# lzhangbj/deep_video_interpolation_extrapolation

Measured on AMD Instinct MI355X. Metric: train frames/s (256x512 len-3 clips), higher is better.
Workload: dtype bf16; 1 GPU; InterNet int_5_len_3 train step 256x512 bf16; per_gpu_batch=8, global_batch=8, parallelism=dp1, step=eager, executor side-stream lanes

## Files before the change

deep_video_interpolation_extrapolation_amd/csrc/conv.hip:

```cpp
#include <cxxabi.h>
#include <dlfcn.h>
#include <stdarg.h>
#include <stdio.h>
#include <stdlib.h>
#include <string.h>

#include <string>
#include <vector>

#include "common.h"

namespace dvie {

static thread_local char g_err[512];
void set_error(const char* fmt, ...) {
  va_list ap;
  va_start(ap, fmt);
  vsnprintf(g_err, sizeof(g_err), fmt, ap);
  va_end(ap);
}
const char* last_error() { return g_err; }

thread_local bool g_trace_on = false;
static thread_local std::vector<const void*> g_trace;
// ... 330 lines not shown
    for (int e = 0; e < 4; ++e) red[tid * 4 + e] = s[e];
    __syncthreads();
    if (tid < 256 / nrl && qb + tid < cq) {
      f32x4 t = f32x4{0.f, 0.f, 0.f, 0.f};
      for (int k = 0; k < nrl; ++k)
        for (int e = 0; e < 4; ++e) t[e] += red[(k * (256 / nrl) + tid) * 4 + e];
      for (int e = 0; e < 4; ++e) p.ws[(long long)blockIdx.x * p.c + 4 * (qb + tid) + e] = t[e];
    }
    __syncthreads();
  }
}

enum { PACK_ELEM = 0, PACK_ROW = 1, PACK_TILE = 2 };
constexpr int PACK_LDS = 8192;
constexpr int PACK_TR = 8, PACK_TC = 64;

__host__ __device__ inline int pack_kind(const dvie_pack_desc& d) {
  if (d.kpad < 64 || d.kpad % 4 != 0) return PACK_ELEM;
  if (d.mode == 0 && d.cin_s * d.kh_s * d.kw_s <= PACK_LDS) return PACK_ROW;
  if (d.mode == 1 && d.kh_s * d.kw_s <= 16 && d.c % 4 == 0) return PACK_TILE;
  return PACK_ELEM;
}

__device__ __forceinline__ void pack_store4(const dvie_pack_desc& p, long long e, const float* v) {
  if (p.dtype == DVIE_BF16) {
    uint2 u;
    u.x = (uint32_t)f2bf(v[0]) | ((uint32_t)f2bf(v[1]) << 16);
    u.y = (uint32_t)f2bf(v[2]) | ((uint32_t)f2bf(v[3]) << 16);
    *(uint2*)((bf16_t*)p.dst + e) = u;
  } else {
    *(f32x4*)((float*)p.dst + e) = f32x4{v[0], v[1], v[2], v[3]};
  }
}

__global__ __launch_bounds__(256) void pack_kernel(const dvie_pack_desc* __restrict__ descs, int n) {
  __shared__ float lds[PACK_LDS];
  int lo = 0, hi = n - 1;
  const int b = blockIdx.x;
  while (lo < hi) {
    const int mid = (lo + hi + 1) >> 1;
    if (descs[mid].blk0 <= b)
      lo = mid;
    else
      hi = mid - 1;
  }
  const dvie_pack_desc p = descs[lo];
  const int lb = b - p.blk0;
  const int ntap = p.th * p.tw, tid = threadIdx.x;
  const int kind = pack_kind(p);

  if (kind == PACK_ROW) {
    const int r = lb, L = p.cin_s * p.kh_s * p.kw_s;
    const bool live = r < p.cout_s;
    for (int i = tid; i < L; i += 256) lds[i] = live ? p.src[(long long)r * L + i] : 0.f;
    __syncthreads();
    for (int k0 = 4 * tid; k0 < p.kpad; k0 += 1024) {
      float v[4];
#pragma unroll
      for (int q = 0; q < 4; ++q) {
        const int k = k0 + q, t = k / p.c, j = k - t * p.c;
        v[q] = 0.f;
        if (live && t < ntap) {
          const int ci = p.cmap ? p.cmap[j] : j;
          const int kh = p.kh0 + (t / p.tw) * p.dkh, kw = p.kw0 + (t % p.tw) * p.dkw;
          if (ci >= 0 && ci < p.cin_s && kh >= 0 && kh < p.kh_s && kw >= 0 && kw < p.kw_s)
            v[q] = lds[(ci * p.kh_s + kh) * p.kw_s + kw];
        }
      }
      pack_store4(p, (long long)r * p.kpad + k0, v);
    }
    return;
  }
  if (kind == PACK_TILE) {
    const int ncb = (p.c + PACK_TC - 1) / PACK_TC;
    const int r0 = (lb / ncb) * PACK_TR, j0 = (lb % ncb) * PACK_TC;
    const int T = p.kh_s * p.kw_s;
    for (int i = tid; i < PACK_TC * PACK_TR * T; i += 256) {
      const int jj = i / (PACK_TR * T), rem = i - jj * (PACK_TR * T), k = rem / T, tp = rem - k * T;
      const int co = j0 + jj, r = r0 + k;
      const int ci = r < p.rows ? (p.cmap ? p.cmap[r] : r) : -1;
      lds[i] = (co < p.cout_s && ci >= 0 && ci < p.cin_s) ? p.src[((long long)co * p.cin_s + ci) * T + tp] : 0.f;
    }
    __syncthreads();
    const int nq = PACK_TC / 4;
    for (int i = tid; i < PACK_TR * ntap * nq; i += 256) {
      const int k = i / (ntap * nq), rem = i - k * (ntap * nq), t = rem / nq, jq = rem - t * nq;
      const int r = r0 + k, j = j0 + 4 * jq;
      if (r >= p.rows || j >= p.c) continue;
      const int kh = p.kh0 + (t / p.tw) * p.dkh, kw = p.kw0 + (t % p.tw) * p.dkw;
      const bool tap_ok = kh >= 0 && kh < p.kh_s && kw >= 0 && kw < p.kw_s;
      float v[4];
#pragma unroll
      for (int q = 0; q < 4; ++q) v[q] = tap_ok ? lds[((j - j0 + q) * PACK_TR + k) * T + kh * p.kw_s + kw] : 0.f;
      pack_store4(p, (long long)r * p.kpad + t * p.c + j, v);
    }
    if (j0 == 0) {
      const int pad = p.kpad - ntap * p.c;
      for (int i = tid; i < PACK_TR * (pad / 4); i += 256) {
        const int k = i / (pad / 4), q4 = i - k * (pad / 4);
        const float z[4] = {0.f, 0.f, 0.f, 0.f};
        if (r0 + k < p.rows) pack_store4(p, (long long)(r0 + k) * p.kpad + ntap * p.c + 4 * q4, z);
      }
    }
    return;
  }
  const long long total = (long long)p.rows * p.kpad;
  const long long e0 = ((long long)lb * 256 + tid) * 4;
  if (e0 >= total) return;
  float v[4];
#pragma unroll
  for (int q = 0; q < 4; ++q) {
    const long long e = e0 + q;
    v[q] = 0.f;
    if (e >= total) continue;
    const int r = (int)(e / p.kpad);
    const int k = (int)(e - (long long)r * p.kpad);
    const int t = k / p.c;
    const int j = k - t * p.c;
    if (t < ntap) {
      int co, ci;
      if (p.mode == 0) {
        co = r;
        ci = p.cmap ? p.cmap[j] : j;
      } else {
        co = j;
        ci = p.cmap ? p.cmap[r] : r;
      }
      const int kh = p.kh0 + (t / p.tw) * p.dkh;
      const int kw = p.kw0 + (t % p.tw) * p.dkw;
      if (co < p.cout_s && ci >= 0 && ci < p.cin_s && kh >= 0 && kh < p.kh_s && kw >= 0 && kw < p.kw_s)
        v[q] = p.src[(((long long)co * p.cin_s + ci) * p.kh_s + kh) * p.kw_s + kw];
    }
  }
  if (e0 + 4 <= total && p.kpad % 4 == 0) {
    pack_store4(p, e0, v);
  } else if (p.dtype == DVIE_BF16) {
    for (int q = 0; q < 4; ++q)
      if (e0 + q < total) ((bf16_t*)p.dst)[e0 + q] = f2bf(v[q]);
  } else {
    for (int q = 0; q < 4; ++q)
      if (e0 + q < total) ((float*)p.dst)[e0 + q] = v[q];
  }
}

}

using namespace dvie;

namespace dvie {
int wgrad_halo_splits(const dvie_wgrad_desc& p);
int wgrad_halo_slabs(const dvie_wgrad_desc& p);
int wgrad_halo_bias_slabs(const dvie_wgrad_desc& p);
bool wgrad_halo_launch(const dvie_wgrad_desc& p, hipStream_t s);
}

extern "C" {

int dvie_wgrad_splits_hint(const dvie_wgrad_desc* d) { return d ? wgrad_halo_splits(*d) : 0; }

int dvie_wgrad_slabs(const dvie_wgrad_desc* d) { return d ? wgrad_halo_slabs(*d) : 0; }

static int colsum_bias_splits(const dvie_wgrad_desc& d) {
  const long long npix = (long long)d.n * d.oh * d.ow;
  const long long s = npix / 512;
  return (int)(s < 1 ? 1 : (s > 2048 ? 2048 : s));
}

static void launch_bias_colsum(const dvie_wgrad_desc& d, hipStream_t s) {
  dvie_colsum_desc c{};
  c.g = d.g;
  c.ws = d.bws;
  c.g_ld = d.g_ld;
  c.rows = (long long)d.n * d.oh * d.ow;
  c.c = d.cout;
  c.splits = colsum_bias_splits(d);
  c.dtype = d.dtype;
  const long long chunk = (c.rows + c.splits - 1) / c.splits;
  if (d.dtype == DVIE_BF16)
    DVIE_LAUNCH(colsum_kernel<bf16_t>, dim3(c.splits), dim3(256), 0, s, c, chunk);
  else
    DVIE_LAUNCH(colsum_kernel<float>, dim3(c.splits), dim3(256), 0, s, c, chunk);
}

int dvie_wgrad_bias_slabs(const dvie_wgrad_desc* d) {
  if (!d) return 0;
  const int h = wgrad_halo_bias_slabs(*d);
  return h > 0 ? h : colsum_bias_splits(*d);
}

int dvie_conv2d_wgrad(const dvie_wgrad_desc* d, void* stream) {
  DVIE_CHECK_ARG(d && d->g && d->x && d->ws, "wgrad: null pointer");
  const int vec = d->dtype == DVIE_BF16 ? 8 : 4;
  DVIE_CHECK_ARG(d->c % vec == 0 && d->g_ld % vec == 0 && d->x_ld % vec == 0,
                 "wgrad: channel alignment c=%d g_ld=%lld x_ld=%lld", d->c, d->g_ld, d->x_ld);
  DVIE_CHECK_ARG(d->splits >= 1, "wgrad: splits");
  const long long npix = (long long)d->n * d->oh * d->ow;
  const int bkp = d->dtype == DVIE_BF16 ? 64 : 32;
  long long chunk = (npix + d->splits - 1) / d->splits;
  chunk = (chunk + bkp - 1) / bkp * bkp;
  dim3 grid((unsigned)d->splits, (unsigned)(((d->cout + 63) / 64) * ((d->c + 63) / 64)), (unsigned)(d->th * d->tw));
  hipStream_t s = (hipStream_t)stream;
  if (d->bws) DVIE_CHECK_ARG(d->cout % 4 == 0 && d->cout <= 4096 && d->g_ld % 4 == 0, "wgrad: bias partials (cout=%d)", d->cout);
  if (wgrad_halo_launch(*d, s)) DVIE_RETURN_LAUNCH();
  DVIE_CHECK_ARG(d->ws_taps == 0, "wgrad: a shared-slab phase launch (ws_taps=%d) needs the halo kernel "
                 "(bf16, stride 1 over the phase view, ow %% 64 == 0)", d->ws_taps);
  if (d->dtype == DVIE_BF16)
    DVIE_LAUNCH(wgrad_kernel<bf16_t>, grid, dim3(256), 0, s, *d, chunk);
  else
    DVIE_LAUNCH(wgrad_kernel<float>, grid, dim3(256), 0, s, *d, chunk);
  if (d->bws) launch_bias_colsum(*d, s);
  DVIE_RETURN_LAUNCH();
}

static int wreduce_check(const dvie_wreduce_desc* d);

int dvie_wgrad_reduce(const dvie_wreduce_desc* d, void* stream) {
  const int rc = wreduce_check(d);
  if (rc != DVIE_OK) return rc;
  const long long total4 = (long long)(d->ws_rows - d->co_off) * d->ws_k / 4;
  if (total4 < 1) return DVIE_OK;
  if (total4 < 2048 && d->splits >= 256)
    DVIE_LAUNCH((wreduce_kernel<4, 64>), dim3((unsigned)((total4 + 3) / 4)), dim3(256), 0, (hipStream_t)stream,
                       *d);
  else
    DVIE_LAUNCH((wreduce_kernel<32, 8>), dim3((unsigned)((total4 + 31) / 32)), dim3(256), 0,
                       (hipStream_t)stream, *d);
  DVIE_RETURN_LAUNCH();
}

static int wreduce_check(const dvie_wreduce_desc* d) {
  DVIE_CHECK_ARG(d && d->ws && d->dw, "wreduce: null pointer");
  DVIE_CHECK_ARG(d->ws_k % 4 == 0 || d->ws_k == 1, "wreduce: ws_k=%d", d->ws_k);
  DVIE_CHECK_ARG(((long long)d->co_off * d->ws_k) % 4 == 0 && d->ws_rows * (long long)d->ws_k % 4 == 0,
                 "wreduce: slab alignment (ws_rows*ws_k and co_off*ws_k multiples of 4)");
  DVIE_CHECK_ARG(d->co_off + d->cout_p <= d->ws_rows, "wreduce: rows");
  return DVIE_OK;
}

int dvie_wgrad_reduce_multi(const dvie_wreduce_desc* descs, int n, void* stream) {
  DVIE_CHECK_ARG(descs && n >= 0, "wreduce_multi: args");
  for (int base = 0; base < n; base += WRM) {
    WreduceMulti m;
    m.n = 0;
    int blocks = 0;
    for (int i = base; i < n && i < base + WRM; ++i) {
      const int rc = wreduce_check(&descs[i]);
      if (rc != DVIE_OK) return rc;
      const long long total4 = (long long)(descs[i].ws_rows - descs[i].co_off) * descs[i].ws_k / 4;
      if (total4 < 1) continue;
      m.d[m.n] = descs[i];
      m.blk0[m.n] = blocks;
      blocks += (int)((total4 + 31) / 32);
      ++m.n;
    }
    m.blk0[m.n] = blocks;
    if (m.n == 0) continue;
    DVIE_LAUNCH(wreduce_multi_kernel, dim3((unsigned)blocks), dim3(256), 0, (hipStream_t)stream, m);
  }
  DVIE_RETURN_LAUNCH();
}

int dvie_colsum(const dvie_colsum_desc* d, void* stream) {
  DVIE_CHECK_ARG(d && d->g && d->ws && d->c % 4 == 0 && d->c <= 4096, "colsum: args");
  DVIE_CHECK_ARG(d->g_ld % 4 == 0, "colsum: g_ld");
  const long long chunk = (d->rows + d->splits - 1) / d->splits;
  hipStream_t s = (hipStream_t)stream;
  if (d->dtype == DVIE_BF16)
    DVIE_LAUNCH(colsum_kernel<bf16_t>, dim3(d->splits), dim3(256), 0, s, *d, chunk);
  else
    DVIE_LAUNCH(colsum_kernel<float>, dim3(d->splits), dim3(256), 0, s, *d, chunk);
  DVIE_RETURN_LAUNCH();
}

int dvie_pack_weights(const dvie_pack_desc* descs_dev, int n, int blocks, void* stream) {
  DVIE_CHECK_ARG(descs_dev && n > 0 && blocks > 0, "pack: args (n %d, blocks %d)", n, blocks);
  DVIE_LAUNCH(pack_kernel, dim3(blocks), dim3(256), 0, (hipStream_t)stream, descs_dev, n);
  DVIE_RETURN_LAUNCH();
}

const char* dvie_last_error(void) { return dvie::last_error(); }

int dvie_pack_blocks(const dvie_pack_desc* d) {
  if (!d || d->rows <= 0 || d->kpad <= 0) return 0;
  switch (pack_kind(*d)) {
    case PACK_ROW: return d->rows;
    case PACK_TILE: return cdiv(d->rows, PACK_TR) * cdiv(d->c, PACK_TC);
    default: return cdiv((long long)d->rows * d->kpad, 1024);
  }
}

int dvie_trace_kernels(int on) {
  const int was = dvie::g_trace_on ? 1 : 0;
  dvie::g_trace_on = on != 0;
  dvie::g_trace.clear();
  return was;
}

const char* dvie_traced_kernels(void) {
  dvie::g_trace_text.clear();
  for (size_t i = 0; i < dvie::g_trace.size(); ++i) {
    if (i) dvie::g_trace_text += ';';
    dvie::g_trace_text += dvie::kernel_name(dvie::g_trace[i]);
  }
  dvie::g_trace.clear();
  return dvie::g_trace_text.c_str();
}

}
```

deep_video_interpolation_extrapolation_amd/csrc/wgrad_halo.hip:

```cpp
#include <stdlib.h>

#include <type_traits>

#include "common.h"


namespace dvie {

typedef __attribute__((address_space(3))) void* lds_ptr_wg;

__device__ __forceinline__ bf16x8 tr_pair(const char* p0, const char* p1) {
  const s16x4 a = __builtin_amdgcn_ds_read_tr16_b64_v4i16((s16x4 __attribute__((address_space(3)))*)p0);
  const s16x4 b = __builtin_amdgcn_ds_read_tr16_b64_v4i16((s16x4 __attribute__((address_space(3)))*)p1);
  typedef short s16x8 __attribute__((ext_vector_type(8)));
  const s16x8 v = {a[0], a[1], a[2], a[3], b[0], b[1], b[2], b[3]};
  return __builtin_bit_cast(bf16x8, v);
}

__device__ __forceinline__ float sum8_bf16(const bf16x8 v, float t) {
  const i32x4 u = __builtin_bit_cast(i32x4, v);
  const bf16x2 one = __builtin_bit_cast(bf16x2, 0x3F803F80);
#pragma unroll
  for (int e = 0; e < 4; ++e) {
    const int w = u[e];
    t = __builtin_amdgcn_fdot2_f32_bf16(__builtin_bit_cast(bf16x2, w), one, t, false);
  }
  return t;
}

template <int TH, int TW, int PR, int TMO, int TMI>
struct WgCfg {
  static constexpr int NT = TH * TW;
  static constexpr int BCO = 64 * TMO, BCI = 64 * TMI;
  static constexpr int HR = PR + TH - 1;
  static constexpr int XW = TW == 1 ? 64 : 72;
  static constexpr int R = HR + PR;
  static constexpr int GROWS = PR * 64;
  static constexpr int GPI = GROWS / 8;
  static constexpr int XPR = XW / 8;
  static constexpr int GSUB = GPI * 1024;
  static constexpr int XSUB = R * XW * 128;
  static constexpr int GSZ = TMO * GSUB, XSZ = TMI * XSUB;
  static constexpr int SMEM = 2 * GSZ + XSZ;
  static constexpr int NACC = NT * TMO * TMI;
};

__device__ __forceinline__ int xcd_chunk(int b, int nb) {
  const int g = b & 7, i = b >> 3;
  const int q = nb >> 3, r = nb & 7;
  return (g < r ? g * (q + 1) : r * (q + 1) + (g - r) * q) + i;
}

template <int TH, int TW, int PR, int TMO, int TMI, int NW = 8, bool PIPE = false, int AB = 0, bool DOB = true,
          bool REUSE = false>
__global__ __launch_bounds__(64 * NW) void wgrad_halo_kernel(const dvie_wgrad_desc p, int n_co, int n_ci, int splits,
                                                             int tiles_x, int tiles_y, int n_tiles, int flags) {
  typedef WgCfg<TH, TW, PR, TMO, TMI> C;
  static_assert(PR % 2 == 0, "row halves");
  static_assert(NW == 8 || (NW == 4 && TMO == 1), "4-wave form: one 32-channel co block");
  static_assert(!REUSE || (PIPE && TMO == 1 && TMI == 1 && TW <= 4), "row-walking form: one fragment per operand");
  __shared__ __attribute__((aligned(1024))) char smem[C::SMEM];
  const int tid = threadIdx.x, lane = tid & 63;
  const int wave = __builtin_amdgcn_readfirstlane(tid >> 6);
  __builtin_assume(wave >= 0 && wave < NW);
  const int merge = flags & 1;
  constexpr int dbg = AB;
  if ((flags & 2) && wave >= NW / 2) __builtin_amdgcn_s_setprio(1);
  const unsigned OOB = 0xFFFFFFF0u;

  const int npair = n_co * n_ci;
  const int lid = xcd_chunk(blockIdx.x, gridDim.x);
  const int pair = lid % npair, split = lid / npair;
  const int cb = pair % n_co, kb = pair / n_co;
  const int c0 = cb * C::BCO, k0 = kb * C::BCI;
  const int t_begin = (int)((long long)split * n_tiles / splits);
  const int t_end = (int)((long long)(split + 1) * n_tiles / splits);

  const unsigned long long gbytes =
      ((unsigned long long)p.n * p.oh * p.ow - 1) * (unsigned long long)p.g_ld * 2ull + (unsigned long long)p.cout * 2ull;
  const unsigned long long xbytes =
      ((unsigned long long)p.n * p.ih * p.iw - 1) * (unsigned long long)p.x_ld * 2ull + (unsigned long long)p.c * 2ull;
  const __amdgpu_buffer_rsrc_t rg = __builtin_amdgcn_make_buffer_rsrc(
      (void*)((const char*)p.g + (size_t)c0 * 2), 0, (int)(gbytes - (unsigned long long)c0 * 2), 0x00020000);
  const __amdgpu_buffer_rsrc_t rx = __builtin_amdgcn_make_buffer_rsrc(
      (void*)((const char*)p.x + (size_t)k0 * 2), 0, (int)(xbytes - (unsigned long long)k0 * 2), 0x00020000);
  const unsigned grow = (unsigned)p.g_ld * 2u, xrow = (unsigned)p.x_ld * 2u;

  const int lrow = lane >> 3, lch = lane & 7;
  const int lcs = lch ^ (((lrow >> 1) & 1) << 2);

  struct TilePos {
    int n, y0, x0, col, ty, tx;
  };
  auto tpos = [&](int t) {
    TilePos q;
    q.ty = t % tiles_y;
    q.col = t / tiles_y;
    q.tx = q.col % tiles_x;
    q.n = q.col / tiles_x;
    q.x0 = q.tx * 64;
    q.y0 = q.ty * PR;
    return q;
  };
  auto tnext = [&](TilePos q) {
    if (++q.ty == tiles_y) {
      q.ty = 0;
      ++q.col;
      if (++q.tx == tiles_x) {
        q.tx = 0;
        ++q.n;
      }
    }
    q.x0 = q.tx * 64;
    q.y0 = q.ty * PR;
    return q;
  };

  constexpr int GQ = (TMO * C::GPI + NW - 1) / NW;
  unsigned gofs[GQ];
  int grd[GQ], grm[GQ];
  bool gok[GQ];
#pragma unroll
  for (int q = 0; q < GQ; ++q) {
    const int pc = wave + NW * q;
    const int sub = pc / C::GPI, pr = pc - sub * C::GPI;
    const int row = pr * 8 + lrow;
    const int ch = 64 * sub + lcs * 8;
    grd[q] = row / 64;
    grm[q] = row & 63;
    gok[q] = pc < TMO * C::GPI && c0 + ch < p.cout;
    gofs[q] = (unsigned)(grd[q] * p.ow + grm[q]) * grow + (unsigned)ch * 2u;
  }
  auto issue_g = [&](const TilePos& T, int gb) {
    char* G = smem + gb * C::GSZ;
    const unsigned base = (unsigned)((T.n * p.oh + T.y0) * p.ow + T.x0) * grow;
    const int ylim = p.oh - T.y0, xlim = p.ow - T.x0;
#pragma unroll
    for (int q = 0; q < GQ; ++q) {
      const int pc = wave + NW * q;
      if (pc < TMO * C::GPI) {
        const unsigned o = (gok[q] && grd[q] < ylim && grm[q] < xlim) ? base + gofs[q] : OOB;
        lds_dma16(rg, G + pc * 1024, o);
      }
    }
  };
  auto issue_x = [&](const TilePos& T, int h0, auto nr) {
    constexpr int npc = decltype(nr)::value * C::XPR;
#pragma unroll 1
    for (int pc = wave; pc < TMI * npc; pc += NW) {
      const int sub = pc / npc, rem = pc - sub * npc;
      const int hrow = h0 + rem / C::XPR, piece = rem - (rem / C::XPR) * C::XPR;
      const int hx = piece * 8 + lrow;
      const int iy = T.y0 + p.dy0 + hrow, ix = T.x0 + p.dx0 + hx;
      const int slot = (T.y0 + hrow) % C::R;
      const int ch = 64 * sub + lcs * 8;
      const bool ok = hx < 64 + TW - 1 && (unsigned)iy < (unsigned)p.ih && (unsigned)ix < (unsigned)p.iw && k0 + ch < p.c;
      const unsigned o = ok ? (unsigned)((T.n * p.ih + iy) * p.iw + ix) * xrow + (unsigned)ch * 2u : OOB;
      char* dst = smem + 2 * C::GSZ + sub * C::XSUB + (slot * C::XW + piece * 8) * 128;
      lds_dma16(rx, dst, o);
    }
  };

  constexpr int XNP = PR * C::XPR;
  constexpr int XQ = (TMI * XNP + NW - 1) / NW;
  unsigned xofs[XQ];
  int xhx[XQ];
  bool xok[XQ];
#pragma unroll
  for (int q = 0; q < XQ; ++q) {
    const int pc = wave + NW * q;
    const int sub = pc / XNP, rem = pc - sub * XNP;
    const int hr = rem / C::XPR, piece = rem - hr * C::XPR;
    const int hx = piece * 8 + lrow;
    const int ch = 64 * sub + lcs * 8;
    xhx[q] = hx;
    xok[q] = pc < TMI * XNP && hx < 64 + TW - 1 && k0 + ch < p.c;
    xofs[q] = (unsigned)(hr * p.iw + hx) * xrow + (unsigned)ch * 2u;
  }
  auto issue_x_new = [&](const TilePos& T) {
    const int h0 = C::HR - PR;
    const int yb = T.y0 + p.dy0 + h0, xb = T.x0 + p.dx0;
    const long long base = ((long long)(T.n * p.ih + yb) * p.iw + xb) * (long long)xrow;
    int ys = (T.y0 + h0) % C::R;
#pragma unroll
    for (int q = 0; q < XQ; ++q) {
      const int pc = wave + NW * q;
      if (pc >= TMI * XNP) continue;
      const int sub = pc / XNP, rem = pc - sub * XNP;
      const int hr = rem / C::XPR, piece = rem - hr * C::XPR;
      int slot = ys + hr;
      slot -= slot >= C::R ? C::R : 0;
      const bool rowok = (unsigned)(yb + hr) < (unsigned)p.ih;
      const bool ok = xok[q] && rowok && (unsigned)(xb + xhx[q]) < (unsigned)p.iw;
      const unsigned o = ok ? (unsigned)(base + (long long)xofs[q]) : OOB;
      char* dst = smem + 2 * C::GSZ + sub * C::XSUB + (slot * C::XW + piece * 8) * 128;
      lds_dma16(rx, dst, o);
    }
  };

  const int grp = lane >> 4, tq = (lane >> 2) & 3, tp = lane & 3;
  auto tr_off = [&](int col0, int m) {
    const int row = m + tq;
    const int col = col0 + 16 * (grp & 1) + 4 * tp;
    const int ch = (col >> 3) ^ (((row >> 1) & 1) << 2);
// ... 582 lines not shown
```

deep_video_interpolation_extrapolation_amd/engine.py:

```python
import ctypes
import math
import os

import torch

from . import _lib as L

PADC = 8
PROFILE = None
DEBUG_NAN = bool(os.environ.get("DVIE_DEBUG_NAN"))
def _wgrad_lane():
    return os.environ.get("DVIE_WGRAD_LANE", "1") != "0"


OP_HOOK = None


def pack_blocks(d):
    n = L.load().dvie_pack_blocks(ctypes.byref(d))
    assert n > 0, "dvie_pack_blocks: empty pack descriptor"
    return n


def _reduce_meta(name, r):
# ... 1308 lines not shown
                    def em(beta, res, res_ld, dact, z, z_ld, src=src, sp=sp, out=out, gout=gout, gld=gld, op=op):
                        o = self.ew_desc(L.EW_MASK, nb, src.H, src.W, src.c, sp, src.buf.C, [(gout, gld, out.H, out.W)],
                                         res=res, res_ld=res_ld, z=z, z_ld=z_ld, dact=dact, beta=beta)
                        o.u.ew.ext_c = int(op.inverse)
                        self.ext_mask = getattr(self, "ext_mask", {})
                        self.ext_mask.setdefault(op.key, []).append(("bwd", len(self.bwd), op))
                        return [o]

                    self._contrib(src, em)
            elif isinstance(op, PoolOp):
                x = op.x
                if x.buf.needs_grad:
                    xp = self.ptr(x, grad=True)

                    def em(beta, res, res_ld, dact, z, z_ld, x=x, xp=xp, out=out, gout=gout, gld=gld):
                        return [self.ew_desc(L.EW_POOLT, nb, x.H, x.W, x.c, xp, x.buf.C, [(gout, gld, out.H, out.W)],
                                             res=res, res_ld=res_ld, z=z, z_ld=z_ld, dact=dact, beta=beta)]

                    self._contrib(x, em)
        for bf in g.buffers:
            if bf.needs_grad and bf.expected and not getattr(bf, "done", False):
                raise RuntimeError(f"incomplete gradient for {bf}: pending {({k: len(v) for k, v in bf.pending.items()})}"
                                   f" of {bf.expected}")

    def _head3_fusable(self, op, gld):
        lay, x, out = op.layer, op.x, op.out
        mode = os.environ.get("DVIE_HEAD3_FUSED", "1")
        if self.dtype != torch.bfloat16 or mode == "0" or (mode == "1" and lay.cout_p != 8):
            return False
        if os.environ.get("DVIE_IM2COL_DGRAD", "0") == "1":
            return False
        if not (lay.trainable and x.buf.needs_grad and op.res is None and lay.kh == 3 and lay.kw == 3
                and lay.stride == 1 and lay.pad == 1 and lay.dil == 1 and lay.cout_p in (8, 24)
                and x.c % 64 == 0 and (out.H, out.W) == (x.H, x.W)):
            return False
        if x.buf.expected.get(x.key(), 0) != 1 or lay.cmap_t is not None and lay.cin != x.c:
            return False
        npx = self.nb * x.H * x.W
        return npx * max(x.buf.C, gld) * 2 < 0xFFFFFF00

    def _head3_ops(self, op, gout, gld, phase, xg, dact):
        lay, x, out = op.layer, op.x, op.out
        nb = self.nb
        ph, wt, kpad = phase
        n_cb = x.c // 64
        splits = max(1, 256 // n_cb)
        slabs = torch.empty(splits * lay.cout_p * 9 * x.c, dtype=torch.float32, device=self.device)
        self.keep.append(slabs)
        o = self._op(L.OP_HEAD3_BWD)
        d = o.u.head3
        d.g, d.h, d.wd, d.dh, d.ws = gout, self.ptr(x), wt.data_ptr(), xg, slabs.data_ptr()
        d.g_ld, d.h_ld, d.dh_ld = gld, x.buf.C, x.buf.C
        d.n, d.hgt, d.wid, d.c = nb, x.H, x.W, x.c
        d.cout, d.kpad, d.dy0, d.dx0 = lay.cout_p, kpad, ph["dy0"], ph["dx0"]
        d.splits, d.dact, d.alpha = splits, dact, 0.2
        npix = nb * x.H * x.W
        o.meta = dict(cls="conv_dgrad", name=lay.name + "+wgrad",
                      flops=2.0 * npix * lay.cout * lay.cin * 9 * 2,
                      bytes=float(self.es * (2 * npix * x.c + npix * lay.cout) + 4 * slabs.numel()))
        ops = [o]
        first = lay not in self.wg_first
        base = len(self.bwd)
        if lay.has_bias:
            csplits = max(1, min(2048, npix // 512))
            c = self._op(L.OP_COLSUM)
            cd = c.u.colsum
            cd.g, cd.ws, cd.g_ld, cd.rows, cd.c, cd.splits, cd.dtype = gout, 0, gld, npix, lay.cout_p, csplits, self.dt
            self.ws_floats = max(self.ws_floats, csplits * lay.cout_p)
            ops.append(c)
        r_op = self._op(L.OP_WREDUCE)
        r = r_op.u.wreduce
        r.ws, r.dw, r.cmap = slabs.data_ptr(), 0, lay.cmap_t.data_ptr()
        r.splits, r.ws_rows, r.ws_k, r.co_off = splits, lay.cout_p, 9 * x.c, 0
        r.cout_p, r.cin_p, r.kh_n, r.kw_n, r.c = lay.cout, lay.cin, lay.kh, lay.kw, x.c
        r.beta = 0 if first else 1
        r_op.ws_ptr = slabs.data_ptr()
        r_op.meta = _reduce_meta(lay.name, r)
        ops.append(r_op)
        self._grad_slots.append((base + len(ops) - 1, lay, "weight", first))
        if lay.has_bias:
            b_op = self._op(L.OP_WREDUCE)
            r = b_op.u.wreduce
            r.ws, r.dw, r.cmap = 0, 0, None
            r.splits, r.ws_rows, r.ws_k, r.co_off = csplits, lay.cout_p, 1, 0
            r.cout_p, r.cin_p, r.kh_n, r.kw_n, r.c = lay.cout, 1, 1, 1, 1
            r.beta = 0 if first else 1
            b_op.meta = _reduce_meta(lay.name + ".bias", r)
            ops.append(b_op)
            self._grad_slots.append((base + len(ops) - 1, lay, "bias", first))
        self.wg_first[lay] = True
        self._uses_left[lay] -= 1
        if self._uses_left[lay] == 0:
            self.completions.append((base + len(ops), lay))
        return ops

    def _conv_backward(self, op, gout, gld):
        lay, x, out = op.layer, op.x, op.out
        nb = self.nb
        npix = nb * out.H * out.W
        taps = lay.fwd_taps()
        head3 = self._head3_fusable(op, gld)
        if lay.trainable and not head3:
            self._emit_wgrad(op, gout, gld)
        if op.res is not None and op.res.buf.needs_grad:
            self._contrib(op.res, None, ident=(gout, gld))
        if x.buf.needs_grad:
            phases = self._dgrad_weights(lay, x.H, x.W)
            xg = self.ptr(x, grad=True)

            def em(beta, res, res_ld, dact, z, z_ld, phases=phases, x=x, xg=xg, out=out, gout=gout, gld=gld, lay=lay):
                if head3:
                    if beta == 0 and res is None and dact in (L.ACT_NONE, L.ACT_LRELU) and \
                            (z is None or z == self.ptr(x)) and len(phases) == 1:
                        return self._head3_ops(op, gout, gld, phases[0], xg, dact)
                    self._emit_wgrad(op, gout, gld)
                ops = []
                if self._im2col_dgrad(lay, x, phases):
                    return self._im2col_dgrad_ops(lay, x, xg, out, gout, gld, phases[0], res, res_ld, z, z_ld, dact,
                                                  beta)
                if self._ph4_eligible(lay, x):
                    wt, kpad = self._dgrad_weights_ph4(lay)
                    taps = dict(th=2, tw=2, dy0=0, dx0=0, ddy=1, ddx=1)
                    o = self.conv_desc(gout, gld, nb, out.H, out.W, lay.cout_p, wt.data_ptr(), kpad, 4 * x.c, out.H,
                                       out.W, 1, 1, taps, xg, x.buf.C, x.H, x.W, osy=2, osx=2, res=res, res_ld=res_ld,
                                       z=z, z_ld=z_ld, dact=dact, beta=beta)
                    o.u.conv.phc = x.c
                    npx = nb * x.H * x.W
                    o.meta = dict(cls="conv_dgrad", name=lay.name,
                                  flops=2.0 * nb * out.H * out.W * lay.cin * lay.cout * 9,
                                  bytes=float(self.es * (nb * out.H * out.W * lay.cout
                                                         + npx * lay.cin * (1 + (res is not None) + (z is not None) + beta)
                                                         + lay.cout * lay.cin * 9)))
                    return [o]
                for ph, wt, kpad in phases:
                    o = self.conv_desc(
                        gout, gld, nb, out.H, out.W, lay.cout_p, wt.data_ptr(), kpad, x.c, ph["oh"], ph["ow"], 1, 1,
                        ph, xg, x.buf.C, x.H, x.W, osy=lay.stride, osx=lay.stride, ory=ph["ry"], orx=ph["rx"],
                        res=res, res_ld=res_ld, z=z, z_ld=z_ld, dact=dact, beta=beta)
                    npx = nb * ph["oh"] * ph["ow"]
                    frac = npx / float(nb * x.H * x.W)
                    o.meta = dict(cls="conv_dgrad",
                                  name=lay.name + (f" [phase {ph['ry']}{ph['rx']}]" if len(phases) > 1 else ""),
                                  flops=2.0 * npx * lay.cin * lay.cout * ph["th"] * ph["tw"],
                                  bytes=float(self.es * (frac * nb * out.H * out.W * lay.cout
                                                         + npx * lay.cin * (1 + (res is not None) + (z is not None) + beta)
                                                         + lay.cout * lay.cin * ph["th"] * ph["tw"])))
                    ops.append(o)
                return ops

            self._contrib(x, em)

    def _wgrad_s2_eligible(self, lay, x, out):
        mode = os.environ.get("DVIE_WGRAD_S2", "1")
        if mode == "1" and x.c < 256:
            return False
        return (self.dtype == torch.bfloat16 and mode != "0" and lay.stride == 2
                and lay.kh == 3 and lay.kw == 3 and lay.pad == 1 and lay.dil == 1 and not lay.transposed
                and x.H % 2 == 0 and x.W % 2 == 0 and out.H == x.H // 2 and out.W == x.W // 2 and out.W % 64 == 0
                and x.c % 8 == 0 and x.buf.C % 8 == 0)

    def _emit_wgrad_s2(self, op, gout, gld):
        lay, x, out = op.layer, op.x, op.out
        nb = self.nb
        npix = nb * out.H * out.W
        lib = L.load()
        ops, slabs, bslabs = [], None, 0
        for a in (0, 1):
            for b in (0, 1):
                o = self._op(L.OP_WGRAD)
                d = o.u.wgrad
                d.g, d.x, d.ws = gout, self.ptr(x) + (a * x.W + b) * x.buf.C * self.es, 0
                d.g_ld, d.x_ld = gld, 2 * x.buf.C
                d.n, d.oh, d.ow, d.cout = nb, out.H, out.W, lay.cout_p
                d.ih, d.iw, d.c, d.sy, d.sx = x.H // 2, x.W, x.c, 1, 1
                d.th, d.tw, d.dy0, d.dx0, d.ddy, d.ddx = 1 + a, 1 + b, -a, -b, 1, 1
                khs, kws = ([1] if a == 0 else [0, 2]), ([1] if b == 0 else [0, 2])
                d.tmap = sum((kh * 3 + kw) << (4 * (i * len(kws) + j)) for i, kh in enumerate(khs)
                             for j, kw in enumerate(kws))
                d.ws_taps = 9
                d.dtype = self.dt
                hint = lib.dvie_wgrad_splits_hint(ctypes.byref(d))
                assert hint > 0, f"{lay.name}: the halo weight-gradient kernel refused a stride-2 phase launch"
                d.splits = hint
                n_s = lib.dvie_wgrad_slabs(ctypes.byref(d))
                assert slabs in (None, n_s), "stride-2 phase launches disagree on their slab count"
                slabs = n_s
                if a == 0 and b == 0 and lay.has_bias:
                    d.bws = 1
                    bslabs = lib.dvie_wgrad_bias_slabs(ctypes.byref(d))
                    d.bws = None
                    o.bws_off = slabs * lay.cout_p * 9 * x.c
                nt = len(khs) * len(kws)
                o.meta = dict(cls="conv_wgrad", name=lay.name + f" [phase {a}{b}]",
                              flops=2.0 * npix * lay.cout * lay.cin * nt,
                              bytes=float(self.es * (npix * lay.cout + npix * lay.cin)
                                          + 4 * slabs * lay.cout_p * nt * x.c))
                ops.append(o)
        wfl = slabs * lay.cout_p * 9 * x.c
        self.ws_floats = max(self.ws_floats, wfl + bslabs * lay.cout_p)
        self.bwd += ops
        self._emit_wreduce(lay, slabs, 9 * x.c, x.c, bslabs, wfl)

    def _emit_wreduce(self, lay, slabs, ws_k, c, bslabs, bias_off):
        o = self._op(L.OP_WREDUCE)
        r = o.u.wreduce
        r.ws, r.dw, r.cmap = 0, 0, lay.cmap_t.data_ptr()
        r.splits, r.ws_rows, r.ws_k, r.co_off = slabs, lay.cout_p, ws_k, 0
        r.cout_p, r.cin_p, r.kh_n, r.kw_n, r.c = lay.cout, lay.cin, lay.kh, lay.kw, c
        first = lay not in self.wg_first
        r.beta = 0 if first else 1
        o.meta = _reduce_meta(lay.name, r)
        self.bwd.append(o)
        self._grad_slots.append((len(self.bwd) - 1, lay, "weight", first))
        if lay.has_bias:
            o = self._op(L.OP_WREDUCE)
            r = o.u.wreduce
            r.ws, r.dw, r.cmap = 0, 0, None
            r.splits, r.ws_rows, r.ws_k, r.co_off = bslabs, lay.cout_p, 1, 0
            r.cout_p, r.cin_p, r.kh_n, r.kw_n, r.c = lay.cout, 1, 1, 1, 1
            r.beta = 0 if first else 1
            o.meta = _reduce_meta(lay.name + ".bias", r)
            o.ws_off = bias_off
            self.bwd.append(o)
            self._grad_slots.append((len(self.bwd) - 1, lay, "bias", first))
        self.wg_first[lay] = True
        self._uses_left[lay] -= 1
        if self._uses_left[lay] == 0:
            self.completions.append((len(self.bwd), lay))

    def _emit_wgrad(self, op, gout, gld):
        lay, x, out = op.layer, op.x, op.out
        if self._wgrad_s2_eligible(lay, x, out) and gld % 8 == 0:
            return self._emit_wgrad_s2(op, gout, gld)
        nb = self.nb
        npix = nb * out.H * out.W
        taps = lay.fwd_taps()
        tiles = rup(lay.cout_p, 64) // 64 * (rup(x.c, 64) // 64)
        ntap = lay.kh * lay.kw
        bkp = 64 if self.dtype == torch.bfloat16 else 32
        splits = max(1, min(max(1, npix // (bkp * 4)), 1024 // max(1, tiles * ntap)))
        o = self._op(L.OP_WGRAD)
        d = o.u.wgrad
        d.g, d.x, d.ws = gout, self.ptr(x), 0
        d.g_ld, d.x_ld = gld, x.buf.C
        d.n, d.oh, d.ow, d.cout = nb, out.H, out.W, lay.cout_p
        d.ih, d.iw, d.c, d.sy, d.sx = x.H, x.W, x.c, lay.stride, lay.stride
        d.th, d.tw, d.dy0, d.dx0, d.ddy, d.ddx = taps["th"], taps["tw"], taps["dy0"], taps["dx0"], taps["ddy"], \
            taps["ddx"]
        d.dtype = self.dt
        lib = L.load()
        hint = lib.dvie_wgrad_splits_hint(ctypes.byref(d))
        d.splits = hint if hint > 0 else splits
        slabs = lib.dvie_wgrad_slabs(ctypes.byref(d))
        wfl = slabs * lay.cout_p * ntap * x.c
        bslabs = 0
        if lay.has_bias:
            d.bws = 1
            bslabs = lib.dvie_wgrad_bias_slabs(ctypes.byref(d))
            d.bws = None
            o.bws_off = wfl
        self.ws_floats = max(self.ws_floats, wfl + bslabs * lay.cout_p)
        o.meta = dict(cls="conv_wgrad", name=lay.name, flops=2.0 * npix * lay.cout * lay.cin * ntap,
                      bytes=float(self.es * (npix * lay.cout + nb * x.H * x.W * lay.cin)
                                  + 4 * slabs * lay.cout_p * ntap * x.c))
        self.bwd.append(o)
        o = self._op(L.OP_WREDUCE)
        r = o.u.wreduce
        r.ws, r.dw, r.cmap = 0, 0, lay.cmap_t.data_ptr()
        r.splits, r.ws_rows, r.ws_k, r.co_off = slabs, lay.cout_p, ntap * x.c, 0
        r.cout_p, r.cin_p, r.kh_n, r.kw_n, r.c = lay.cout, lay.cin, lay.kh, lay.kw, x.c
        first = lay not in self.wg_first
        r.beta = 0 if first else 1
        o.meta = _reduce_meta(lay.name, r)
        self.bwd.append(o)
        self._grad_slots.append((len(self.bwd) - 1, lay, "weight", first))
        if lay.has_bias:
            o = self._op(L.OP_WREDUCE)
            r = o.u.wreduce
            r.ws, r.dw, r.cmap = 0, 0, None
            r.splits, r.ws_rows, r.ws_k, r.co_off = bslabs, lay.cout_p, 1, 0
            r.cout_p, r.cin_p, r.kh_n, r.kw_n, r.c = lay.cout, 1, 1, 1, 1
            r.beta = 0 if first else 1
            o.meta = _reduce_meta(lay.name + ".bias", r)
            o.ws_off = wfl
            self.bwd.append(o)
            self._grad_slots.append((len(self.bwd) - 1, lay, "bias", first))
        self.wg_first[lay] = True
        self._uses_left[lay] -= 1
        if self._uses_left[lay] == 0:
            self.completions.append((len(self.bwd), lay))

    def _im2col_dgrad(self, lay, x, phases):
        if self.dtype != torch.bfloat16 or os.environ.get("DVIE_IM2COL_DGRAD", "0") != "1":
            return False
        if lay.stride != 1 or len(phases) != 1:
            return False
        ph, _, kpad = phases[0]
        return (ph["th"] * ph["tw"] > 1 and lay.cout_p % 8 == 0 and lay.cout_p <= 32 and x.c >= 128
                and kpad % 64 == 0 and ph["ry"] == 0 and ph["rx"] == 0)

    def _im2col_dgrad_ops(self, lay, x, xg, out, gout, gld, phase, res, res_ld, z, z_ld, dact, beta):
        ph, wt, kpad = phase
        nb = self.nb
        npx = nb * ph["oh"] * ph["ow"]
        buf = self.__dict__.get("_i2c")
        if buf is None or buf.numel() < npx * kpad:
            buf = torch.empty(npx * kpad, dtype=self.dtype, device=self.device)
            self._i2c = buf
            self.keep.append(buf)
# ... 460 lines not shown
```

Baseline: 254.6 frames/s.

## Add dedicated stride-2 3x3 wgrad kernel with row-ring LDS reuse

```diff
diff --git a/deep_video_interpolation_extrapolation_amd/csrc/conv.hip b/deep_video_interpolation_extrapolation_amd/csrc/conv.hip
--- a/deep_video_interpolation_extrapolation_amd/csrc/conv.hip
+++ b/deep_video_interpolation_extrapolation_amd/csrc/conv.hip
@@ -506,11 +506,18 @@
 int wgrad_halo_slabs(const dvie_wgrad_desc& p);
 int wgrad_halo_bias_slabs(const dvie_wgrad_desc& p);
 bool wgrad_halo_launch(const dvie_wgrad_desc& p, hipStream_t s);
+int wgrad_s2_splits(const dvie_wgrad_desc& p);
+int wgrad_s2_bias_slabs(const dvie_wgrad_desc& p);
+bool wgrad_s2_launch(const dvie_wgrad_desc& p, hipStream_t s);
 }
 
 extern "C" {
 
-int dvie_wgrad_splits_hint(const dvie_wgrad_desc* d) { return d ? wgrad_halo_splits(*d) : 0; }
+int dvie_wgrad_splits_hint(const dvie_wgrad_desc* d) {
+  if (!d) return 0;
+  const int h = wgrad_halo_splits(*d);
+  return h > 0 ? h : wgrad_s2_splits(*d);
+}
 
 int dvie_wgrad_slabs(const dvie_wgrad_desc* d) { return d ? wgrad_halo_slabs(*d) : 0; }
 
@@ -538,7 +545,8 @@
 
 int dvie_wgrad_bias_slabs(const dvie_wgrad_desc* d) {
   if (!d) return 0;
-  const int h = wgrad_halo_bias_slabs(*d);
+  int h = wgrad_halo_bias_slabs(*d);
+  if (h <= 0) h = wgrad_s2_bias_slabs(*d);
   return h > 0 ? h : colsum_bias_splits(*d);
 }
 
@@ -556,6 +564,7 @@
   hipStream_t s = (hipStream_t)stream;
   if (d->bws) DVIE_CHECK_ARG(d->cout % 4 == 0 && d->cout <= 4096 && d->g_ld % 4 == 0, "wgrad: bias partials (cout=%d)", d->cout);
   if (wgrad_halo_launch(*d, s)) DVIE_RETURN_LAUNCH();
+  if (wgrad_s2_launch(*d, s)) DVIE_RETURN_LAUNCH();
   DVIE_CHECK_ARG(d->ws_taps == 0, "wgrad: a shared-slab phase launch (ws_taps=%d) needs the halo kernel "
                  "(bf16, stride 1 over the phase view, ow %% 64 == 0)", d->ws_taps);
   if (d->dtype == DVIE_BF16)
diff --git a/deep_video_interpolation_extrapolation_amd/csrc/wgrad_frag.h b/deep_video_interpolation_extrapolation_amd/csrc/wgrad_frag.h
--- /dev/null
+++ b/deep_video_interpolation_extrapolation_amd/csrc/wgrad_frag.h
@@ -0,0 +1,31 @@
+#pragma once
+#include "common.h"
+
+namespace dvie {
+
+__device__ __forceinline__ bf16x8 tr_pair(const char* p0, const char* p1) {
+  const s16x4 a = __builtin_amdgcn_ds_read_tr16_b64_v4i16((s16x4 __attribute__((address_space(3)))*)p0);
+  const s16x4 b = __builtin_amdgcn_ds_read_tr16_b64_v4i16((s16x4 __attribute__((address_space(3)))*)p1);
+  typedef short s16x8 __attribute__((ext_vector_type(8)));
+  const s16x8 v = {a[0], a[1], a[2], a[3], b[0], b[1], b[2], b[3]};
+  return __builtin_bit_cast(bf16x8, v);
+}
+
+__device__ __forceinline__ float sum8_bf16(const bf16x8 v, float t) {
+  const i32x4 u = __builtin_bit_cast(i32x4, v);
+  const bf16x2 one = __builtin_bit_cast(bf16x2, 0x3F803F80);
+#pragma unroll
+  for (int e = 0; e < 4; ++e) {
+    const int w = u[e];
+    t = __builtin_amdgcn_fdot2_f32_bf16(__builtin_bit_cast(bf16x2, w), one, t, false);
+  }
+  return t;
+}
+
+__device__ __forceinline__ int xcd_chunk(int b, int nb) {
+  const int g = b & 7, i = b >> 3;
+  const int q = nb >> 3, r = nb & 7;
+  return (g < r ? g * (q + 1) : r * (q + 1) + (g - r) * q) + i;
+}
+
+}
diff --git a/deep_video_interpolation_extrapolation_amd/csrc/wgrad_halo.hip b/deep_video_interpolation_extrapolation_amd/csrc/wgrad_halo.hip
--- a/deep_video_interpolation_extrapolation_amd/csrc/wgrad_halo.hip
+++ b/deep_video_interpolation_extrapolation_amd/csrc/wgrad_halo.hip
@@ -3,30 +3,11 @@
 #include <type_traits>
 
 #include "common.h"
-
+#include "wgrad_frag.h"
 
 namespace dvie {
 
 typedef __attribute__((address_space(3))) void* lds_ptr_wg;
-
-__device__ __forceinline__ bf16x8 tr_pair(const char* p0, const char* p1) {
-  const s16x4 a = __builtin_amdgcn_ds_read_tr16_b64_v4i16((s16x4 __attribute__((address_space(3)))*)p0);
-  const s16x4 b = __builtin_amdgcn_ds_read_tr16_b64_v4i16((s16x4 __attribute__((address_space(3)))*)p1);
-  typedef short s16x8 __attribute__((ext_vector_type(8)));
-  const s16x8 v = {a[0], a[1], a[2], a[3], b[0], b[1], b[2], b[3]};
-  return __builtin_bit_cast(bf16x8, v);
-}
-
-__device__ __forceinline__ float sum8_bf16(const bf16x8 v, float t) {
-  const i32x4 u = __builtin_bit_cast(i32x4, v);
-  const bf16x2 one = __builtin_bit_cast(bf16x2, 0x3F803F80);
-#pragma unroll
-  for (int e = 0; e < 4; ++e) {
-    const int w = u[e];
-    t = __builtin_amdgcn_fdot2_f32_bf16(__builtin_bit_cast(bf16x2, w), one, t, false);
-  }
-  return t;
-}
 
 template <int TH, int TW, int PR, int TMO, int TMI>
 struct WgCfg {
@@ -45,11 +26,6 @@
   static constexpr int NACC = NT * TMO * TMI;
 };
 
-__device__ __forceinline__ int xcd_chunk(int b, int nb) {
-  const int g = b & 7, i = b >> 3;
-  const int q = nb >> 3, r = nb & 7;
-  return (g < r ? g * (q + 1) : r * (q + 1) + (g - r) * q) + i;
-}
 
 template <int TH, int TW, int PR, int TMO, int TMI, int NW = 8, bool PIPE = false, int AB = 0, bool DOB = true,
           bool REUSE = false>
diff --git a/deep_video_interpolation_extrapolation_amd/csrc/wgrad_s2.hip b/deep_video_interpolation_extrapolation_amd/csrc/wgrad_s2.hip
--- /dev/null
+++ b/deep_video_interpolation_extrapolation_amd/csrc/wgrad_s2.hip
@@ -0,0 +1,304 @@
+#include <stdlib.h>
+
+#include "common.h"
+#include "wgrad_frag.h"
+
+namespace dvie {
+
+constexpr int S2_D = 2;
+constexpr int S2_RX = 2 * S2_D + 3;
+constexpr int S2_RG = S2_D + 1;
+constexpr int S2_OPC = 9, S2_EPC = 8;
+constexpr int S2_XPC = S2_OPC + S2_EPC;
+constexpr int S2_XROW = S2_XPC * 1024;
+constexpr int S2_GROW = 8 * 1024;
+constexpr int S2_XRING = S2_RX * S2_XROW;
+constexpr int S2_RING = S2_XRING + S2_RG * S2_GROW;
+constexpr int S2_NPC = 8 + 2 * S2_XPC;
+constexpr int S2_PQ = (S2_NPC + 7) / 8;
+constexpr int S2_PARK = 4 * 9 * 1024 * 4;
+constexpr int S2_SMEM = S2_RING > S2_PARK ? S2_RING : S2_PARK;
+static_assert(S2_SMEM <= 160 * 1024, "LDS of a CU");
+static_assert(S2_NPC % 8 != 0 && S2_PQ * (S2_D - 1) < 16, "the two vmcnt constants below");
+
+#define DVIE_WS2_VMCNT_LGKM0(N) __builtin_amdgcn_s_waitcnt(((N) & 15) | (((N) >> 4) << 14) | (7 << 4))
+
+template <bool DOB>
+__global__ __launch_bounds__(512) void wgrad_s2_kernel(const dvie_wgrad_desc p, int n_co, int n_ci, int splits,
+                                                       int tiles_x, int n_rows) {
+  __shared__ __attribute__((aligned(1024))) char smem[S2_SMEM];
+  const int tid = threadIdx.x, lane = tid & 63;
+  const int wave = __builtin_amdgcn_readfirstlane(tid >> 6);
+  __builtin_assume(wave >= 0 && wave < 8);
+  const unsigned OOB = 0xFFFFFFF0u;
+
+  const int npair = n_co * n_ci;
+  const int lid = xcd_chunk(blockIdx.x, gridDim.x);
+  const int pair = lid % npair, split = lid / npair;
+  const int cb = pair % n_co, kb = pair / n_co;
+  const int c0 = cb * 64, k0 = kb * 64;
+  const int r_begin = (int)((long long)split * n_rows / splits);
+  const int r_end = (int)((long long)(split + 1) * n_rows / splits);
+
+  const unsigned long long gbytes =
+      ((unsigned long long)p.n * p.oh * p.ow - 1) * (unsigned long long)p.g_ld * 2ull + (unsigned long long)p.cout * 2ull;
+  const unsigned long long xbytes =
+      ((unsigned long long)p.n * p.ih * p.iw - 1) * (unsigned long long)p.x_ld * 2ull + (unsigned long long)p.c * 2ull;
+  const __amdgpu_buffer_rsrc_t rg = __builtin_amdgcn_make_buffer_rsrc(
+      (void*)((const char*)p.g + (size_t)c0 * 2), 0, (int)(gbytes - (unsigned long long)c0 * 2), 0x00020000);
+  const __amdgpu_buffer_rsrc_t rx = __builtin_amdgcn_make_buffer_rsrc(
+      (void*)((const char*)p.x + (size_t)k0 * 2), 0, (int)(xbytes - (unsigned long long)k0 * 2), 0x00020000);
+  const unsigned grow = (unsigned)p.g_ld * 2u, xrow = (unsigned)p.x_ld * 2u;
+
+  const int lrow = lane >> 3, lch = lane & 7;
+  const int lcs = lch ^ (((lrow >> 1) & 1) << 2);
+  const bool g_chok = c0 + lcs * 8 < p.cout, x_chok = k0 + lcs * 8 < p.c;
+
+  auto x_col = [&](int pp, int& dx, bool& has) {
+    if (pp < S2_OPC) {
+      const int j = pp * 8 + lrow;
+      dx = 2 * j - 1;
+      has = j < 65;
+    } else {
+      dx = 2 * ((pp - S2_OPC) * 8 + lrow);
+      has = true;
+    }
+  };
+
+  unsigned lofs[S2_PQ];
+  int lcol[S2_PQ];
+  bool lok[S2_PQ];
+#pragma unroll
+  for (int q = 0; q < S2_PQ; ++q) {
+    const int pc = wave + 8 * q;
+    if (pc < 8) {
+      lcol[q] = pc * 8 + lrow;
+      lok[q] = g_chok;
+      lofs[q] = (unsigned)lcol[q] * grow + (unsigned)lcs * 16u;
+    } else {
+      const int xp = pc - 8, rs = xp / S2_XPC, pp = xp - rs * S2_XPC;
+      int dx;
+      bool has;
+      x_col(pp, dx, has);
+      lcol[q] = dx;
+      lok[q] = has && x_chok && pc < S2_NPC;
+      lofs[q] = (unsigned)(rs * p.iw + dx) * xrow + (unsigned)lcs * 16u;
+    }
+  }
+
+  struct RowPos {
+    int n, tx, oy;
+  };
+  auto rnext = [&](RowPos r) {
+    if (++r.oy == p.oh) {
+      r.oy = 0;
+      if (++r.tx == tiles_x) {
+        r.tx = 0;
+        ++r.n;
+      }
+    }
+    return r;
+  };
+  auto issue_row = [&](const RowPos& R, bool live, int sg, int sx) {
+    const int x0 = R.tx * 64;
+    const unsigned gbase = ((unsigned)(R.n * p.oh + R.oy) * (unsigned)p.ow + (unsigned)x0) * grow;
+    const unsigned xbase = ((unsigned)(R.n * p.ih + 2 * R.oy) * (unsigned)p.iw + 2u * (unsigned)x0) * xrow;
+    const int glim = p.ow - x0;
+    const int sx1 = sx + 1 == S2_RX ? 0 : sx + 1;
+#pragma unroll
+    for (int q = 0; q < S2_PQ; ++q) {
+      const int pc = wave + 8 * q;
+      if (pc >= S2_NPC) continue;
+      if (pc < 8) {
+        const bool ok = live && lok[q] && lcol[q] < glim;
+        lds_dma16(rg, smem + S2_XRING + sg * S2_GROW + pc * 1024, ok ? gbase + lofs[q] : OOB);
+      } else {
+        const int xp = pc - 8, rs = xp / S2_XPC, pp = xp - rs * S2_XPC;
+        const bool ok = live && lok[q] && (unsigned)(2 * x0 + lcol[q]) < (unsigned)p.iw;
+        lds_dma16(rx, smem + (rs ? sx1 : sx) * S2_XROW + pp * 1024, ok ? xbase + lofs[q] : OOB);
+      }
+    }
+  };
+
+  const int grp = lane >> 4, tq = (lane >> 2) & 3, tp = lane & 3;
+  auto tr_off = [&](int col0, int m) {
+    const int row = m + tq;
+    const int col = col0 + 16 * (grp & 1) + 4 * tp;
+    const int ch = (col >> 3) ^ (((row >> 1) & 1) << 2);
+    return row * 128 + ch * 16 + (col & 7) * 2 + 8 * 128 * (grp >> 1);
+  };
+  const int wco = (wave >> 1) & 1, wci = wave & 1, whalf = wave >> 2;
+  const int g_off = tr_off(wco * 32, 0) + whalf * (32 * 128);
+  const int x_off0 = tr_off(wci * 32, 0) + whalf * (32 * 128);
+  const int x_off1 = tr_off(wci * 32, 1) + whalf * (32 * 128);
+
+  f32x16 acc[9];
+#pragma unroll
+  for (int a = 0; a < 9; ++a)
+#pragma unroll
+    for (int e = 0; e < 16; ++e) acc[a][e] = 0.f;
+  const bool dob = DOB && kb == 0 && wci == 0;
+  float bsum = 0.f;
+
+  if (r_begin < r_end) {
+    RowPos Ri;
+    Ri.oy = r_begin % p.oh;
+    const int col = r_begin / p.oh;
+    Ri.tx = col % tiles_x;
+    Ri.n = col / tiles_x;
+    int coy = Ri.oy;
+    if (Ri.oy > 0) {
+      const unsigned xbase = (unsigned)((Ri.n * p.ih + 2 * Ri.oy - 1) * p.iw + 2 * Ri.tx * 64) * xrow;
+#pragma unroll 1
+      for (int pp = wave; pp < S2_XPC; pp += 8) {
+        int dx;
+        bool has;
+        x_col(pp, dx, has);
+        const bool ok = has && x_chok && (unsigned)(2 * Ri.tx * 64 + dx) < (unsigned)p.iw;
+        lds_dma16(rx, smem + (S2_RX - 1) * S2_XROW + pp * 1024, ok ? xbase + (unsigned)dx * xrow + (unsigned)lcs * 16u : OOB);
+      }
+    }
+    int isg = 0, isx = 0, ri = r_begin;
+#pragma unroll
+    for (int d = 0; d < S2_D; ++d) {
+      issue_row(Ri, ri < r_end, isg, isx);
+      Ri = rnext(Ri);
+      ++ri;
+      isg = isg + 1 == S2_RG ? 0 : isg + 1;
+      isx = isx + 2 >= S2_RX ? isx + 2 - S2_RX : isx + 2;
+    }
+    int csg = 0, csx = 0, cpx = S2_RX - 1;
+    for (int r = r_begin; r < r_end; ++r) {
+      if (wave < S2_NPC % 8)
+        DVIE_WS2_VMCNT_LGKM0((S2_D - 1) * S2_PQ);
+      else
+        DVIE_WS2_VMCNT_LGKM0((S2_D - 1) * (S2_PQ - 1));
+      __builtin_amdgcn_s_barrier();
+      issue_row(Ri, ri < r_end, isg, isx);
+      Ri = rnext(Ri);
+      ++ri;
+      isg = isg + 1 == S2_RG ? 0 : isg + 1;
+      isx = isx + 2 >= S2_RX ? isx + 2 - S2_RX : isx + 2;
+
+      const char* G = smem + S2_XRING + csg * S2_GROW + g_off;
+      const int csx1 = csx + 1 == S2_RX ? 0 : csx + 1;
+      const char* Xr[3] = {smem + cpx * S2_XROW, smem + csx * S2_XROW, smem + csx1 * S2_XROW};
+      const bool top = coy > 0;
+#pragma unroll
+      for (int c = 0; c < 2; ++c) {
+        const int pb = c * (16 * 128);
+        const bf16x8 ga = tr_pair(G + pb, G + pb + 4 * 128);
+#pragma unroll
+        for (int ti = 0; ti < 3; ++ti) {
+          if (ti == 0 && !top) continue;
+          const char* X = Xr[ti] + pb;
+          const bf16x8 b0 = tr_pair(X + x_off0, X + x_off0 + 4 * 128);
+          const bf16x8 b1 = tr_pair(X + S2_OPC * 1024 + x_off0, X + S2_OPC * 1024 + x_off0 + 4 * 128);
+          const bf16x8 b2 = tr_pair(X + x_off1, X + x_off1 + 4 * 128);
+          acc[3 * ti + 0] = __builtin_amdgcn_mfma_f32_32x32x16_bf16(ga, b0, acc[3 * ti + 0], 0, 0, 0);
+          acc[3 * ti + 1] = __builtin_amdgcn_mfma_f32_32x32x16_bf16(ga, b1, acc[3 * ti + 1], 0, 0, 0);
+          acc[3 * ti + 2] = __builtin_amdgcn_mfma_f32_32x32x16_bf16(ga, b2, acc[3 * ti + 2], 0, 0, 0);
+        }
+        if constexpr (DOB) bsum = sum8_bf16(ga, bsum);
+      }
+      if (++coy == p.oh) coy = 0;
+      cpx = csx1;
+      csg = csg + 1 == S2_RG ? 0 : csg + 1;
+      csx = csx + 2 >= S2_RX ? csx + 2 - S2_RX : csx + 2;
+    }
+  }
+  __builtin_amdgcn_s_waitcnt(0);
+  __syncthreads();
+
+  if (dob) {
+    const float t = bsum + __shfl_xor(bsum, 32, 64);
+    const int co = c0 + wco * 32 + (lane & 31);
+    if (lane < 32 && co < p.cout) p.bws[(long long)(2 * split + whalf) * p.cout + co] = t;
+  }
+
+  const long long ws_k = 9ll * p.c;
+  const int r32 = lane & 31, hh = lane >> 5;
+  float* slab = p.ws + (long long)split * p.cout * ws_k;
+  constexpr int TO = 5;
+  float* park = (float*)smem + (wco * 2 + wci) * (9 * 1024) + lane;
+#pragma unroll
+  for (int t = 0; t < 9; ++t)
+    if ((t < TO) != (whalf == 0)) {
+#pragma unroll
+      for (int e = 0; e < 16; ++e) park[t * 1024 + e * 64] = acc[t][e];
+    }
+  __syncthreads();
+  const int ci = k0 + wci * 32 + r32;
+  const int cob = c0 + wco * 32;
+#pragma unroll
+  for (int t = 0; t < 9; ++t) {
+    if ((t < TO) != (whalf == 0)) continue;
+    float v[16];
+#pragma unroll
+    for (int e = 0; e < 16; ++e) v[e] = acc[t][e] + park[t * 1024 + e * 64];
+    if (ci >= p.c) continue;
+    float* dst = slab + (long long)(cob + 4 * hh) * ws_k + (long long)t * p.c + ci;
+    if (cob + 32 <= p.cout) {
+#pragma unroll
+      for (int e = 0; e < 16; ++e) dst[(long long)(8 * (e >> 2) + (e & 3)) * ws_k] = v[e];
+    } else {
+#pragma unroll
+      for (int e = 0; e < 16; ++e)
+        if (cob + 4 * hh + 8 * (e >> 2) + (e & 3) < p.cout) dst[(long long)(8 * (e >> 2) + (e & 3)) * ws_k] = v[e];
+    }
+  }
+}
+
+static bool wgrad_s2_on() {
+  const char* e = getenv("DVIE_WGRAD_S2K");
+  return !(e && *e == '0');
+}
+
+static bool wgrad_s2_eligible(const dvie_wgrad_desc& p) {
+  if (p.dtype != DVIE_BF16 || !wgrad_s2_on()) return false;
+  if (p.th != 3 || p.tw != 3 || p.sy != 2 || p.sx != 2 || p.ddy != 1 || p.ddx != 1 || p.dy0 != -1 || p.dx0 != -1) return false;
+  if (p.ws_taps != 0) return false;
+  if (p.n < 1 || p.oh < 1 || p.ow < 1 || p.ih != 2 * p.oh || p.iw != 2 * p.ow) return false;
+  if (p.c < 8 || p.cout < 8 || p.c % 8 != 0 || p.cout % 8 != 0 || p.g_ld % 8 != 0 || p.x_ld % 8 != 0) return false;
+  const unsigned long long npx = (unsigned long long)p.n * p.ih * p.iw, npg = (unsigned long long)p.n * p.oh * p.ow;
+  if (npx >= (1ull << 31) || npg >= (1ull << 31)) return false;
+  const unsigned long long xspan = ((npx - 1) * (unsigned long long)p.x_ld + (unsigned long long)p.c) * 2ull;
+  const unsigned long long gspan = ((npg - 1) * (unsigned long long)p.g_ld + (unsigned long long)p.cout) * 2ull;
+  if (xspan >= 0xFFFFFF00ull || gspan >= 0xFFFFFF00ull) return false;
+  return true;
+}
+
+static void wgrad_s2_rows(const dvie_wgrad_desc& p, int& tiles_x, long long& n_rows, int& n_co, int& n_ci) {
+  tiles_x = (p.ow + 63) / 64;
+  n_rows = (long long)p.n * tiles_x * p.oh;
+  n_co = (p.cout + 63) / 64;
+  n_ci = (p.c + 63) / 64;
+}
+
+int wgrad_s2_splits(const dvie_wgrad_desc& p) {
+  if (!wgrad_s2_eligible(p)) return 0;
+  int tx, nco, nci;
+  long long nr;
+  wgrad_s2_rows(p, tx, nr, nco, nci);
+  long long s = 256 / (nco * nci);
+  if (s > nr) s = nr;
+  return (int)(s < 1 ? 1 : s);
+}
+
+int wgrad_s2_bias_slabs(const dvie_wgrad_desc& p) { return wgrad_s2_eligible(p) ? 2 * p.splits : 0; }
+
+bool wgrad_s2_launch(const dvie_wgrad_desc& p, hipStream_t s) {
+  if (!wgrad_s2_eligible(p)) return false;
+  int tiles_x, n_co, n_ci;
+  long long n_rows;
+  wgrad_s2_rows(p, tiles_x, n_rows, n_co, n_ci);
+  const long long grid = (long long)n_co * n_ci * p.splits;
+  if (grid >= (1ll << 31)) return false;
+  if (p.bws)
+    DVIE_LAUNCH(wgrad_s2_kernel<true>, dim3((unsigned)grid), dim3(512), 0, s, p, n_co, n_ci, p.splits, tiles_x, (int)n_rows);
+  else
+    DVIE_LAUNCH(wgrad_s2_kernel<false>, dim3((unsigned)grid), dim3(512), 0, s, p, n_co, n_ci, p.splits, tiles_x, (int)n_rows);
+  return true;
+}
+
+}
diff --git a/deep_video_interpolation_extrapolation_amd/engine.py b/deep_video_interpolation_extrapolation_amd/engine.py
--- a/deep_video_interpolation_extrapolation_amd/engine.py
+++ b/deep_video_interpolation_extrapolation_amd/engine.py
@@ -1484,9 +1484,7 @@
 
     def _wgrad_s2_eligible(self, lay, x, out):
         mode = os.environ.get("DVIE_WGRAD_S2", "1")
-        if mode == "1" and x.c < 256:
-            return False
-        return (self.dtype == torch.bfloat16 and mode != "0" and lay.stride == 2
+        return (self.dtype == torch.bfloat16 and mode == "2" and lay.stride == 2
                 and lay.kh == 3 and lay.kw == 3 and lay.pad == 1 and lay.dil == 1 and not lay.transposed
                 and x.H % 2 == 0 and x.W % 2 == 0 and out.H == x.H // 2 and out.W == x.W // 2 and out.W % 64 == 0
                 and x.c % 8 == 0 and x.buf.C % 8 == 0)
```

After: 257.0 frames/s, median of 6. No clear change (+1.0%).
